# zhirui-gao/Curve-Gaussian

Hardware: AMD Instinct MI355X
Metric: Msplats rasterized/s (fwd+bwd) (higher is better)
Workload: dtype f32

## Files before the change

### curve_gaussian_amd/csrc/curve_math.h

```cpp
#pragma once
#include "kernels.h"

namespace cgs {

constexpr int NORM_SLOTS = 64;
constexpr int NQ_FWD = 3, NQ_ALL = 5;
constexpr int NORM_WORDS = NQ_ALL * NORM_SLOTS;
static_assert(NORM_WORDS <= 384, "norms buffer layout");

struct SampleCoef {
    float c[4];
    float cf[4];
    float d[3];
    float l[2];
    float lf[2];
    float pad;
};
static_assert(sizeof(SampleCoef) == 64, "SampleCoef must be 16 floats");

struct V3 { float x, y, z; };
__device__ __forceinline__ V3 operator+(V3 a, V3 b) { return {a.x + b.x, a.y + b.y, a.z + b.z}; }
__device__ __forceinline__ V3 operator-(V3 a, V3 b) { return {a.x - b.x, a.y - b.y, a.z - b.z}; }
__device__ __forceinline__ V3 operator*(float s, V3 a) { return {s * a.x, s * a.y, s * a.z}; }
__device__ __forceinline__ float dot(V3 a, V3 b) { return a.x * b.x + a.y * b.y + a.z * b.z; }
__device__ __forceinline__ V3 cross(V3 a, V3 b) { return {a.y * b.z - a.z * b.y, a.z * b.x - a.x * b.z, a.x * b.y - a.y * b.x}; }

struct CurveCP { V3 p0, p1, p2, p3; bool bez; };
__device__ __forceinline__ CurveCP load_curve(const float* __restrict__ cp, const uint8_t* __restrict__ is_bezier, int b) {
    const float4* q = reinterpret_cast<const float4*>(cp + (size_t)b * 12);
    const float4 a = q[0], c = q[1], d = q[2];
    CurveCP r;
    r.p0 = {a.x, a.y, a.z}; r.p1 = {a.w, c.x, c.y}; r.p2 = {c.z, c.w, d.x}; r.p3 = {d.y, d.z, d.w};
    r.bez = is_bezier ? (is_bezier[b] != 0) : true;
    return r;
}
__device__ __forceinline__ V3 curve_tangent(const CurveCP& c, const SampleCoef& k) {
    if (!c.bez) return c.p3 - c.p0;
    return k.d[0] * (c.p1 - c.p0) + k.d[1] * (c.p2 - c.p1) + k.d[2] * (c.p3 - c.p2);
}

struct BlockConst {
    float N1, N2, D2, D1;
};
__device__ __forceinline__ void stage_consts(const SampleCoef* __restrict__ coef, int m, const double* __restrict__ norms,
                                             SampleCoef* s_coef, BlockConst* s_bc) {
    const float* src = reinterpret_cast<const float*>(coef);
    float* dst = reinterpret_cast<float*>(s_coef);
    for (int t = threadIdx.x; t < m * 16; t += blockDim.x) dst[t] = src[t];
    __shared__ double s_q[NQ_ALL];
    for (int base = 0; base < NQ_ALL * NORM_SLOTS; base += blockDim.x) {
        const int idx = base + threadIdx.x;
        double v = idx < NQ_ALL * NORM_SLOTS ? norms[idx] : 0.0;
#pragma unroll
        for (int off = NORM_SLOTS / 2; off >= 1; off >>= 1) v += __shfl_xor(v, off, 64);
        if (idx < NQ_ALL * NORM_SLOTS && (idx % NORM_SLOTS) == 0) s_q[idx / NORM_SLOTS] = v;
    }
    __syncthreads();
    if (threadIdx.x == 0) {
        const double N1 = sqrt(s_q[0]), N2 = sqrt(s_q[1]) / N1;
        s_bc->N1 = (float)N1;
        s_bc->N2 = (float)N2;
        s_bc->D2 = (float)s_q[3];
        s_bc->D1 = (float)(s_q[4] - s_q[3] / (N2 * N2 * N2) * (s_q[2] / N1));
    }
    __syncthreads();
}
constexpr int SAMPLE_BLOCK = 256;
constexpr int MAX_M = 32;

struct CurveLaunch { int cpb; dim3 grid; };
inline CurveLaunch curve_launch(int B, int m) {
    const int cpb = SAMPLE_BLOCK / m;
    return {cpb, dim3((B + cpb - 1) / cpb)};
}
struct CurveSlot { int i, b; bool valid; };
__device__ __forceinline__ CurveSlot curve_slot(int B, int m, int curves_per_block) {
    const int lc = threadIdx.x / m;
    CurveSlot t;
    t.i = threadIdx.x - lc * m;
    t.b = blockIdx.x * curves_per_block + lc;
    t.valid = lc < curves_per_block && t.b < B;
    return t;
}

template <int N>
__device__ __forceinline__ void block_accumulate(const double (&v)[N], double* norms, int q0) {
    __shared__ double s_part[N][4];
    double w[N];
#pragma unroll
    for (int k = 0; k < N; k++) w[k] = (double)wave_sum((float)v[k]);
    const int wave = threadIdx.x >> 6;
    if ((threadIdx.x & 63) == 0) {
#pragma unroll
        for (int k = 0; k < N; k++) s_part[k][wave] = w[k];
    }
    __syncthreads();
    if (threadIdx.x < N) {
        double t = 0;
        for (int wv = 0; wv < (int)(blockDim.x >> 6); wv++) t += s_part[threadIdx.x][wv];
        atomicAdd(norms + (q0 + threadIdx.x) * NORM_SLOTS + (blockIdx.x % NORM_SLOTS), t);
    }
}

struct QuatFwd { float a[4], qa[4], N[4], D; int k; bool flip; };
__device__ __forceinline__ float sel4(const float (&arr)[4], int k) {
    return k == 0 ? arr[0] : (k == 1 ? arr[1] : (k == 2 ? arr[2] : arr[3]));
}
__device__ __forceinline__ QuatFwd quat_forward(const float M[3][3], float q[4]) {
    QuatFwd f;
    const float m00 = M[0][0], m01 = M[0][1], m02 = M[0][2], m10 = M[1][0], m11 = M[1][1], m12 = M[1][2], m20 = M[2][0],
                m21 = M[2][1], m22 = M[2][2];
    f.a[0] = 1.0f + m00 + m11 + m22; f.a[1] = 1.0f + m00 - m11 - m22;
    f.a[2] = 1.0f - m00 + m11 - m22; f.a[3] = 1.0f - m00 - m11 + m22;
    int k = 0;
#pragma unroll
    for (int j = 0; j < 4; j++) f.qa[j] = f.a[j] > 0.f ? sqrtf(f.a[j]) : 0.f;
    float qak = f.qa[0];
#pragma unroll
    for (int j = 1; j < 4; j++) {
        const bool gt = f.qa[j] > qak;
        k = gt ? j : k;
        qak = gt ? f.qa[j] : qak;
    }
    f.k = k;
    const float sq = qak * qak;
    if (k == 0) { f.N[0] = sq; f.N[1] = m21 - m12; f.N[2] = m02 - m20; f.N[3] = m10 - m01; }
    else if (k == 1) { f.N[0] = m21 - m12; f.N[1] = sq; f.N[2] = m10 + m01; f.N[3] = m02 + m20; }
    else if (k == 2) { f.N[0] = m02 - m20; f.N[1] = m10 + m01; f.N[2] = sq; f.N[3] = m12 + m21; }
    else { f.N[0] = m10 - m01; f.N[1] = m20 + m02; f.N[2] = m21 + m12; f.N[3] = sq; }
    f.D = 2.0f * fmaxf(qak, 0.1f);
#pragma unroll
    for (int j = 0; j < 4; j++) q[j] = f.N[j] / f.D;
    f.flip = q[0] < 0.f;
    if (f.flip) {
#pragma unroll
        for (int j = 0; j < 4; j++) q[j] = -q[j];
    }
    return f;
}
__device__ __forceinline__ void quat_backward(const QuatFwd& f, const float g_out[4], float gM[3][3]) {
    float gc[4], gN[4];
    float gD = 0.f;
#pragma unroll
    for (int j = 0; j < 4; j++) {
        gc[j] = f.flip ? -g_out[j] : g_out[j];
        gN[j] = gc[j] / f.D;
        gD -= gc[j] * f.N[j] / (f.D * f.D);
    }
    const int k = f.k;
    const float qak = sel4(f.qa, k);
    const float g_qa = (qak > 0.1f ? 2.f * gD : 0.f) + sel4(gN, k) * 2.f * qak;
    const float g_a = sel4(f.a, k) > 0.f ? g_qa / (2.f * qak) : 0.f;
#pragma unroll
    for (int r = 0; r < 3; r++)
#pragma unroll
        for (int c = 0; c < 3; c++) gM[r][c] = 0.f;
    const float s00 = (k == 0 || k == 1) ? 1.f : -1.f, s11 = (k == 0 || k == 2) ? 1.f : -1.f,
                s22 = (k == 0 || k == 3) ? 1.f : -1.f;
    gM[0][0] = s00 * g_a; gM[1][1] = s11 * g_a; gM[2][2] = s22 * g_a;
    if (k == 0) {
        gM[2][1] += gN[1]; gM[1][2] -= gN[1]; gM[0][2] += gN[2]; gM[2][0] -= gN[2]; gM[1][0] += gN[3]; gM[0][1] -= gN[3];
    } else if (k == 1) {
        gM[2][1] += gN[0]; gM[1][2] -= gN[0]; gM[1][0] += gN[2]; gM[0][1] += gN[2]; gM[0][2] += gN[3]; gM[2][0] += gN[3];
    } else if (k == 2) {
        gM[0][2] += gN[0]; gM[2][0] -= gN[0]; gM[1][0] += gN[1]; gM[0][1] += gN[1]; gM[1][2] += gN[3]; gM[2][1] += gN[3];
    } else {
        gM[1][0] += gN[0]; gM[0][1] -= gN[0]; gM[2][0] += gN[1]; gM[0][2] += gN[1]; gM[2][1] += gN[2]; gM[1][2] += gN[2];
    }
}

struct SampleFwd {
    V3 xyz, dvec, tan, v0, c1v, v1, c2v, v2;
    float dist, n;
};
__device__ __forceinline__ SampleFwd sample_forward(const CurveCP& c, const SampleCoef& k, float N1, float N2, float eps) {
    SampleFwd s;
    V3 front;
    if (c.bez) {
        s.xyz = k.c[0] * c.p0 + k.c[1] * c.p1 + k.c[2] * c.p2 + k.c[3] * c.p3;
        front = k.cf[0] * c.p0 + k.cf[1] * c.p1 + k.cf[2] * c.p2 + k.cf[3] * c.p3;
    } else {
        s.xyz = k.l[0] * c.p0 + k.l[1] * c.p3;
        front = k.lf[0] * c.p0 + k.lf[1] * c.p3;
    }
    s.dvec = s.xyz - front;
    s.dist = sqrtf(dot(s.dvec, s.dvec));
    s.tan = curve_tangent(c, k);
    s.n = sqrtf(dot(s.tan, s.tan));
    s.v0 = {s.tan.x / (s.n + eps), s.tan.y / (s.n + eps), s.tan.z / (s.n + eps)};
    s.c1v = {s.tan.y, -s.tan.x, 0.f};
    s.v1 = {s.c1v.x / N1, s.c1v.y / N1, 0.f};
    s.c2v = cross(s.tan, s.v1);
    s.v2 = {s.c2v.x / N2, s.c2v.y / N2, s.c2v.z / N2};
    return s;
}
__device__ __forceinline__ void rot_matrix(const SampleFwd& s, float M[3][3]) {
    M[0][0] = s.v0.x; M[0][1] = s.v1.x; M[0][2] = s.v2.x;
    M[1][0] = s.v0.y; M[1][1] = s.v1.y; M[1][2] = s.v2.y;
    M[2][0] = s.v0.z; M[2][1] = s.v1.z; M[2][2] = s.v2.z;
}

struct NormTerms { double d2, a; };
__device__ __forceinline__ NormTerms norm_sum_terms(const SampleFwd& s, float N2, V3 g_v1, V3 g_v2) {
    NormTerms t;
    t.d2 = (double)dot(g_v2, s.c2v);
    t.a = (double)dot(g_v1, s.c1v) + (double)((1.f / N2) * dot(cross(g_v2, s.tan), s.c1v));
    return t;
}

struct CurveGrad { V3 gp0, gp1, gp2, gp3; float gw; };
__device__ __forceinline__ CurveGrad sample_backward_tail(const CurveCP& c, const SampleCoef& k, const SampleFwd& s, float w, float eps,
                                                          float N1, float N2, float D2, float D1, V3 g_v0, V3 g_v1, V3 g_v2, V3 g_x,
                                                          bool has_scaling, V3 g_scl) {
    CurveGrad o;
    o.gp0 = o.gp1 = o.gp2 = o.gp3 = V3{0.f, 0.f, 0.f};
    o.gw = 0.f;
    const float iN2 = 1.f / N2;
    const V3 g_c2v = iN2 * g_v2 - (D2 * iN2 * iN2 * iN2) * s.c2v;
    V3 g_tan = cross(s.v1, g_c2v);
    const V3 g_v1t = g_v1 + cross(g_c2v, s.tan);
    const float iN1 = 1.f / N1;
    const V3 g_c1v = iN1 * g_v1t - (D1 * iN1 * iN1 * iN1) * s.c1v;
    g_tan.y += g_c1v.x;
    g_tan.x -= g_c1v.y;
    if (s.n > 0.f) {
        const float ne = s.n + eps;
        const float coefv = dot(g_v0, s.tan) / (s.n * ne * ne);
        g_tan = g_tan + (1.f / ne) * g_v0 - coefv * s.tan;
    } else {
        g_tan = g_tan + (1.f / eps) * g_v0;
    }
    V3 g_front = {0, 0, 0};
    if (has_scaling) {
        const float gd = g_scl.x;
        o.gw = (g_scl.y + g_scl.z) * w;
        if (s.dist > 0.f) {
            const V3 gdv = (gd / s.dist) * s.dvec;
            g_x = g_x + gdv;
            g_front = {-gdv.x, -gdv.y, -gdv.z};
        }
    }
    if (c.bez) {
        o.gp0 = k.c[0] * g_x + k.cf[0] * g_front - k.d[0] * g_tan;
        o.gp1 = k.c[1] * g_x + k.cf[1] * g_front + (k.d[0] - k.d[1]) * g_tan;
        o.gp2 = k.c[2] * g_x + k.cf[2] * g_front + (k.d[1] - k.d[2]) * g_tan;
        o.gp3 = k.c[3] * g_x + k.cf[3] * g_front + k.d[2] * g_tan;
    } else {
        o.gp0 = k.l[0] * g_x + k.lf[0] * g_front - g_tan;
        o.gp3 = k.l[1] * g_x + k.lf[1] * g_front + g_tan;
    }
    return o;
}
constexpr int CURVE_PART = 13;
template <typename F>
__device__ __forceinline__ void curve_reduce(const CurveGrad& g, float (*s_part)[256 + 1], int B, int m, int curves_per_block, F fn) {
    const int t = threadIdx.x;
    s_part[0][t] = g.gp0.x; s_part[1][t] = g.gp0.y; s_part[2][t] = g.gp0.z;
    s_part[3][t] = g.gp1.x; s_part[4][t] = g.gp1.y; s_part[5][t] = g.gp1.z;
    s_part[6][t] = g.gp2.x; s_part[7][t] = g.gp2.y; s_part[8][t] = g.gp2.z;
    s_part[9][t] = g.gp3.x; s_part[10][t] = g.gp3.y; s_part[11][t] = g.gp3.z;
    s_part[12][t] = g.gw;
    __syncthreads();
    for (int o = threadIdx.x; o < curves_per_block * CURVE_PART; o += blockDim.x) {
        const int c2 = o / CURVE_PART, f = o - c2 * CURVE_PART;
        float sum = 0.f;
        for (int q = 0; q < m; q++) sum += s_part[f][c2 * m + q];
        const int bb = blockIdx.x * curves_per_block + c2;
        if (bb < B) fn(bb, f, sum);
    }
}
__device__ __forceinline__ void store_curve_grad(float* __restrict__ g_cp, float* __restrict__ g_width, int bb, int f, float v,
                                                 int accumulate) {
    float* dst = f < 12 ? g_cp + (size_t)bb * 12 + f : g_width + bb;
    *dst = accumulate ? *dst + v : v;
}

__device__ __forceinline__ float sigmoidf_(float x) { return 1.f / (1.f + expf(-x)); }

struct AttrsFwd { float4 rot_n; float opac, mk; float4 all_map; float nrm; };
__device__ __forceinline__ AttrsFwd attrs_forward(const float4 q, const V3 x, float opacity_logit, bool has_mask,
                                                  float mask_logit, float mask_thr, const V3 cam,
                                                  const float* __restrict__ vm) {
    AttrsFwd o;
    const float op = sigmoidf_(opacity_logit);
    o.nrm = sqrtf(q.x * q.x + q.y * q.y + q.z * q.z + q.w * q.w);
    const float den = fmaxf(o.nrm, 1e-12f);
    const float r = q.x / den, qi = q.y / den, qj = q.z / den, qk = q.w / den;
    o.rot_n = make_float4(r, qi, qj, qk);
    o.mk = 1.f;
    if (has_mask) o.mk = sigmoidf_(mask_logit) > mask_thr ? 1.f : 0.f;
    o.opac = op * o.mk;
    const float two_s = 2.0f / (r * r + qi * qi + qj * qj + qk * qk);
    V3 d = {1.f - two_s * (qj * qj + qk * qk), two_s * (qi * qj + qk * r), two_s * (qi * qk - qj * r)};
    if (dot(d, cam - x) < 0.0f) d = {-d.x, -d.y, -d.z};
    o.all_map = make_float4(d.x * vm[0] + d.y * vm[4] + d.z * vm[8], d.x * vm[1] + d.y * vm[5] + d.z * vm[9],
                            d.x * vm[2] + d.y * vm[6] + d.z * vm[10], 1.0f);
    return o;
}

struct AttrsBwd { float4 g_rot_raw; float g_op_term, g_mask_logit, mk; };
__device__ __forceinline__ AttrsBwd attrs_backward(const float4 q, const V3 x, float opacity_logit, bool has_mask,
                                                   float mask_logit, float mask_thr, const V3 cam,
                                                   const float* __restrict__ vm, float4 gqn, bool has_ga, const float4 ga,
                                                   float go, bool has_gs, const V3 gs, const V3 scaling) {
    AttrsBwd o;
    const float op = sigmoidf_(opacity_logit);
    const float nrm = sqrtf(q.x * q.x + q.y * q.y + q.z * q.z + q.w * q.w);
    const float den = fmaxf(nrm, 1e-12f);
    const float r = q.x / den, qi = q.y / den, qj = q.z / den, qk = q.w / den;
    float gq[4] = {gqn.x, gqn.y, gqn.z, gqn.w};
    if (has_ga) {
        V3 gd = {vm[0] * ga.x + vm[1] * ga.y + vm[2] * ga.z, vm[4] * ga.x + vm[5] * ga.y + vm[6] * ga.z,
                 vm[8] * ga.x + vm[9] * ga.y + vm[10] * ga.z};
        const float s2 = r * r + qi * qi + qj * qj + qk * qk;
        const float two_s = 2.0f / s2;
        const V3 d = {1.f - two_s * (qj * qj + qk * qk), two_s * (qi * qj + qk * r), two_s * (qi * qk - qj * r)};
        if (dot(d, cam - x) < 0.0f) gd = {-gd.x, -gd.y, -gd.z};
        const float e0 = qj * qj + qk * qk, e1 = qi * qj + qk * r, e2 = qi * qk - qj * r;
        const float g_two_s = -gd.x * e0 + gd.y * e1 + gd.z * e2;
        const float g_s2 = g_two_s * (-2.0f / (s2 * s2));
        gq[0] += two_s * (gd.y * qk - gd.z * qj) + g_s2 * 2.f * r;
        gq[1] += two_s * (gd.y * qj + gd.z * qk) + g_s2 * 2.f * qi;
        gq[2] += two_s * (-2.f * gd.x * qj + gd.y * qi - gd.z * r) + g_s2 * 2.f * qj;
        gq[3] += two_s * (-2.f * gd.x * qk + gd.y * r + gd.z * qi) + g_s2 * 2.f * qk;
    }
    if (nrm > 1e-12f) {
        const float dq = gq[0] * r + gq[1] * qi + gq[2] * qj + gq[3] * qk;
        o.g_rot_raw = make_float4((gq[0] - r * dq) / nrm, (gq[1] - qi * dq) / nrm, (gq[2] - qj * dq) / nrm, (gq[3] - qk * dq) / nrm);
    } else {
        o.g_rot_raw = make_float4(gq[0] / 1e-12f, gq[1] / 1e-12f, gq[2] / 1e-12f, gq[3] / 1e-12f);
    }
    float sg = 0.f;
    o.mk = 1.f;
    if (has_mask) {
        sg = sigmoidf_(mask_logit);
        o.mk = sg > mask_thr ? 1.f : 0.f;
    }
    o.g_op_term = go * o.mk * op * (1.f - op);
    float g_mask = go * op;
    if (has_gs) g_mask += gs.x * scaling.x + gs.y * scaling.y + gs.z * scaling.z;
    o.g_mask_logit = has_mask ? g_mask * sg * (1.f - sg) : 0.f;
    return o;
}

__device__ __forceinline__ void quat_grad_to_axes(const SampleFwd& s, const float4 gq, V3& g_v0, V3& g_v1, V3& g_v2) {
    float M[3][3], q[4], gM[3][3];
    rot_matrix(s, M);
    const QuatFwd f = quat_forward(M, q);
    const float go[4] = {gq.x, gq.y, gq.z, gq.w};
    quat_backward(f, go, gM);
    g_v0 = {gM[0][0], gM[1][0], gM[2][0]};
    g_v1 = {gM[0][1], gM[1][1], gM[2][1]};
    g_v2 = {gM[0][2], gM[1][2], gM[2][2]};
}

}
```

### curve_gaussian_amd/csrc/sampling.hip

```cpp
#include <algorithm>

#include "curve_math.h"

namespace cgs {

constexpr int F12_BLOCK = 1024;
__global__ void __launch_bounds__(F12_BLOCK) k_sample_f12(int B, int m, const float* __restrict__ cp,
                                                         const uint8_t* __restrict__ is_bezier,
                                                         const SampleCoef* __restrict__ coef, double* __restrict__ norms) {
    __shared__ SampleCoef s_coef[MAX_M];
    __shared__ double s_part[3][F12_BLOCK / 64];
    const float* src = reinterpret_cast<const float*>(coef);
    float* dst = reinterpret_cast<float*>(s_coef);
    for (int t = threadIdx.x; t < m * 16; t += blockDim.x) dst[t] = src[t];
    __syncthreads();
    double a1 = 0, a2 = 0, a3 = 0;
    for (int p = blockIdx.x * blockDim.x + threadIdx.x; p < B * m; p += gridDim.x * blockDim.x) {
        const int b = p / m, i = p - b * m;
        const CurveCP c = load_curve(cp, is_bezier, b);
        const V3 t = curve_tangent(c, s_coef[i]);
        const V3 c1 = {t.y, -t.x, 0.f};
        const V3 x = cross(t, c1);
        a1 += (double)(t.y * t.y + t.x * t.x);
        a2 += (double)(x.x * x.x + x.y * x.y + x.z * x.z);
        a3 += (double)dot(cross(x, t), c1);
    }
#pragma unroll
    for (int off = 32; off >= 1; off >>= 1) {
        a1 += __shfl_xor(a1, off, 64);
        a2 += __shfl_xor(a2, off, 64);
        a3 += __shfl_xor(a3, off, 64);
    }
    if ((threadIdx.x & 63) == 0) {
        s_part[0][threadIdx.x >> 6] = a1; s_part[1][threadIdx.x >> 6] = a2; s_part[2][threadIdx.x >> 6] = a3;
    }
    __syncthreads();
    if (threadIdx.x < 3) {
        double t = 0;
        for (int wv = 0; wv < (int)(blockDim.x >> 6); wv++) t += s_part[threadIdx.x][wv];
        norms[threadIdx.x * NORM_SLOTS + blockIdx.x] = t;
    } else if (threadIdx.x < NQ_ALL) {
        norms[threadIdx.x * NORM_SLOTS + blockIdx.x] = 0.0;
    }
}

__global__ void __launch_bounds__(256) k_sample_f3(int B, int m, const float* __restrict__ cp,
                                                   const float* __restrict__ width,
                                                   const uint8_t* __restrict__ is_bezier,
                                                   const SampleCoef* __restrict__ coef, float eps,
                                                   const double* __restrict__ norms, float* __restrict__ xyz,
                                                   float* __restrict__ rot, float* __restrict__ scaling) {
    __shared__ SampleCoef s_coef[MAX_M];
    __shared__ BlockConst s_bc;
    stage_consts(coef, m, norms, s_coef, &s_bc);
    const int p = blockIdx.x * blockDim.x + threadIdx.x;
    if (p >= B * m) return;
    const int b = p / m, i = p - b * m;
    const float N1 = s_bc.N1, N2 = s_bc.N2;
    const CurveCP c = load_curve(cp, is_bezier, b);
    const float w = expf(width[b]);
    const SampleFwd s = sample_forward(c, s_coef[i], N1, N2, eps);
    float M[3][3], q[4];
    rot_matrix(s, M);
    quat_forward(M, q);
    xyz[3 * p] = s.xyz.x; xyz[3 * p + 1] = s.xyz.y; xyz[3 * p + 2] = s.xyz.z;
    reinterpret_cast<float4*>(rot)[p] = make_float4(q[0], q[1], q[2], q[3]);
    scaling[3 * p] = s.dist; scaling[3 * p + 1] = w; scaling[3 * p + 2] = w;
}

__global__ void __launch_bounds__(SAMPLE_BLOCK) k_sample_bwd_sums(int B, int m, const float* __restrict__ cp,
                                                                  const uint8_t* __restrict__ is_bezier,
                                                                  const SampleCoef* __restrict__ coef, float eps,
                                                                  double* __restrict__ norms, const float* __restrict__ g_rot,
                                                                  float* __restrict__ gv_cache) {
    __shared__ SampleCoef s_coef[MAX_M];
    __shared__ BlockConst s_bc;
    stage_consts(coef, m, norms, s_coef, &s_bc);
    const int p = blockIdx.x * blockDim.x + threadIdx.x;
    NormTerms t = {0, 0};
    if (g_rot && p < B * m) {
        const int b = p / m, i = p - b * m;
        const SampleFwd s = sample_forward(load_curve(cp, is_bezier, b), s_coef[i], s_bc.N1, s_bc.N2, eps);
        V3 g_v0, g_v1, g_v2;
        quat_grad_to_axes(s, reinterpret_cast<const float4*>(g_rot)[p], g_v0, g_v1, g_v2);
        float* gv = gv_cache + p;
        const size_t PS = (size_t)B * m;
        gv[0] = g_v0.x; gv[PS] = g_v0.y; gv[2 * PS] = g_v0.z; gv[3 * PS] = g_v1.x; gv[4 * PS] = g_v1.y; gv[5 * PS] = g_v1.z;
        gv[6 * PS] = g_v2.x; gv[7 * PS] = g_v2.y; gv[8 * PS] = g_v2.z;
        t = norm_sum_terms(s, s_bc.N2, g_v1, g_v2);
    }
    const double acc[2] = {t.d2, t.a};
    block_accumulate<2>(acc, norms, 3);
}

__global__ void __launch_bounds__(SAMPLE_BLOCK) k_sample_bwd_curves(int B, int m, int curves_per_block,
                                                                    const float* __restrict__ cp,
                                                                    const float* __restrict__ width,
                                                                    const uint8_t* __restrict__ is_bezier,
                                                                    const SampleCoef* __restrict__ coef, float eps,
                                                                    const double* __restrict__ norms,
                                                                    const float* __restrict__ g_xyz, bool has_rot,
                                                                    const float* __restrict__ g_scaling,
                                                                    float* __restrict__ g_cp, float* __restrict__ g_width,
                                                                    const float* __restrict__ gv_cache) {
    __shared__ float s_part[CURVE_PART][SAMPLE_BLOCK + 1];
    __shared__ SampleCoef s_coef[MAX_M];
    __shared__ BlockConst s_bc;
    stage_consts(coef, m, norms, s_coef, &s_bc);
    const CurveSlot t = curve_slot(B, m, curves_per_block);
    CurveGrad cg = {};
    if (t.valid) {
        const CurveCP c = load_curve(cp, is_bezier, t.b);
        const SampleCoef k = s_coef[t.i];
        const size_t p = (size_t)t.b * m + t.i;
        const SampleFwd s = sample_forward(c, k, s_bc.N1, s_bc.N2, eps);
        V3 g_v0 = {0, 0, 0}, g_v1 = {0, 0, 0}, g_v2 = {0, 0, 0}, g_x = {0, 0, 0}, g_s = {0, 0, 0};
        if (has_rot) {
            const float* gv = gv_cache + p;
            const size_t PS = (size_t)B * m;
            g_v0 = {gv[0], gv[PS], gv[2 * PS]}; g_v1 = {gv[3 * PS], gv[4 * PS], gv[5 * PS]}; g_v2 = {gv[6 * PS], gv[7 * PS], gv[8 * PS]};
        }
        if (g_xyz) g_x = {g_xyz[3 * p], g_xyz[3 * p + 1], g_xyz[3 * p + 2]};
        if (g_scaling) g_s = {g_scaling[3 * p], g_scaling[3 * p + 1], g_scaling[3 * p + 2]};
        cg = sample_backward_tail(c, k, s, expf(width[t.b]), eps, s_bc.N1, s_bc.N2, s_bc.D2, s_bc.D1, g_v0, g_v1, g_v2, g_x,
                                  g_scaling != nullptr, g_s);
    }
    curve_reduce(cg, s_part, B, m, curves_per_block, [&](int bb, int f, float sum) { store_curve_grad(g_cp, g_width, bb, f, sum, 0); });
}

__global__ void __launch_bounds__(SAMPLE_BLOCK) k_sample_bwd_close(int B, int m, int curves_per_block, const float* __restrict__ cp,
                                                                   const float* __restrict__ width,
                                                                   const uint8_t* __restrict__ is_bezier,
                                                                   const SampleCoef* __restrict__ coef, float eps,
                                                                   const double* __restrict__ norms, const float* __restrict__ part,
                                                                   float* __restrict__ g_cp, float* __restrict__ g_width,
                                                                   int accumulate) {
    __shared__ float s_part[CURVE_PART][SAMPLE_BLOCK + 1];
    __shared__ SampleCoef s_coef[MAX_M];
    __shared__ BlockConst s_bc;
    stage_consts(coef, m, norms, s_coef, &s_bc);
    const CurveSlot t = curve_slot(B, m, curves_per_block);
    CurveGrad cg = {};
    if (t.valid) {
        const CurveCP c = load_curve(cp, is_bezier, t.b);
        const SampleCoef k = s_coef[t.i];
        const SampleFwd s = sample_forward(c, k, s_bc.N1, s_bc.N2, eps);
        const V3 z = {0.f, 0.f, 0.f};
        cg = sample_backward_tail(c, k, s, expf(width[t.b]), eps, s_bc.N1, s_bc.N2, s_bc.D2, s_bc.D1, z, z, z, z, false, z);
    }
    curve_reduce(cg, s_part, B, m, curves_per_block, [&](int bb, int f, float sum) {
        store_curve_grad(g_cp, g_width, bb, f, part[(size_t)bb * CURVE_PART + f] + sum, accumulate);
    });
}


__global__ void __launch_bounds__(256) k_attrs_fwd(int B, int m, const float* __restrict__ rot_raw,
                                                   const float* __restrict__ xyz,
                                                   const float* __restrict__ opacity_logit,
                                                   const float* __restrict__ mask_logit, float mask_thr,
                                                   const float* __restrict__ scaling,
                                                   const float* __restrict__ campos, const float* __restrict__ vm,
                                                   float* __restrict__ rot_n, float* __restrict__ opac,
                                                   float* __restrict__ scl_out, float* __restrict__ all_map) {
    const int p = blockIdx.x * blockDim.x + threadIdx.x;
    if (p >= B * m) return;
    const int b = p / m;
    const V3 cam = {campos[0], campos[1], campos[2]};
    const float4 q = reinterpret_cast<const float4*>(rot_raw)[p];
    const V3 x = {xyz[3 * p], xyz[3 * p + 1], xyz[3 * p + 2]};
    const AttrsFwd a = attrs_forward(q, x, opacity_logit[b], mask_logit != nullptr, mask_logit ? mask_logit[p] : 0.f, mask_thr,
                                     cam, vm);
    reinterpret_cast<float4*>(rot_n)[p] = a.rot_n;
    opac[p] = a.opac;
    if (scl_out) {
        scl_out[3 * p] = scaling[3 * p] * a.mk; scl_out[3 * p + 1] = scaling[3 * p + 1] * a.mk;
        scl_out[3 * p + 2] = scaling[3 * p + 2] * a.mk;
    }
    reinterpret_cast<float4*>(all_map)[p] = a.all_map;
}

__global__ void __launch_bounds__(SAMPLE_BLOCK) k_attrs_bwd(
    int B, int m, int curves_per_block, const float* __restrict__ rot_raw, const float* __restrict__ xyz,
    const float* __restrict__ opacity_logit, const float* __restrict__ mask_logit, float mask_thr,
    const float* __restrict__ scaling, const float* __restrict__ campos, const float* __restrict__ vm,
    const float* __restrict__ g_rot_n, const float* __restrict__ g_opac, const float* __restrict__ g_scl_out,
    const float* __restrict__ g_all_map, float* __restrict__ g_rot_raw, float* __restrict__ g_opacity_logit,
    float* __restrict__ g_mask_logit, float* __restrict__ g_scaling) {
    __shared__ float s_go[SAMPLE_BLOCK];
    const CurveSlot t = curve_slot(B, m, curves_per_block);
    const int b = t.b;
    float g_op_term = 0.f;
    if (t.valid) {
        const size_t p = (size_t)b * m + t.i;
        const V3 cam = {campos[0], campos[1], campos[2]};
        const float4 q = reinterpret_cast<const float4*>(rot_raw)[p];
        const V3 x = {xyz[3 * p], xyz[3 * p + 1], xyz[3 * p + 2]};
        const float4 gqn = g_rot_n ? reinterpret_cast<const float4*>(g_rot_n)[p] : make_float4(0.f, 0.f, 0.f, 0.f);
        const float4 ga = g_all_map ? reinterpret_cast<const float4*>(g_all_map)[p] : make_float4(0.f, 0.f, 0.f, 0.f);
        V3 gs = {0.f, 0.f, 0.f}, sc = {0.f, 0.f, 0.f};
        if (g_scl_out) {
            gs = {g_scl_out[3 * p], g_scl_out[3 * p + 1], g_scl_out[3 * p + 2]};
            sc = {scaling[3 * p], scaling[3 * p + 1], scaling[3 * p + 2]};
        }
        const AttrsBwd o = attrs_backward(q, x, opacity_logit[b], mask_logit != nullptr, mask_logit ? mask_logit[p] : 0.f,
                                          mask_thr, cam, vm, gqn, g_all_map != nullptr, ga, g_opac ? g_opac[p] : 0.f,
                                          g_scl_out != nullptr, gs, sc);
        reinterpret_cast<float4*>(g_rot_raw)[p] = o.g_rot_raw;
        g_op_term = o.g_op_term;
        if (g_scl_out && g_scaling) { g_scaling[3 * p] = gs.x * o.mk; g_scaling[3 * p + 1] = gs.y * o.mk; g_scaling[3 * p + 2] = gs.z * o.mk; }
        if (g_mask_logit) g_mask_logit[p] = o.g_mask_logit;
    }
    s_go[threadIdx.x] = g_op_term;
    __syncthreads();
    if (t.valid && t.i == 0) {
        float sum = 0.f;
        for (int q = 0; q < m; q++) sum += s_go[threadIdx.x + q];
        g_opacity_logit[b] = sum;
    }
}

static int f12_threads(long long P) { return P <= 128 * 1024 ? 256 : (P <= 600 * 1024 ? 512 : 1024); }

void launch_sample_norms(hipStream_t s, int B, int m, const float* cp, const uint8_t* is_bezier, const void* coef, double* norms) {
    ProfScope p("sample_f12", s);
    hipLaunchKernelGGL(k_sample_f12, dim3(NORM_SLOTS), dim3(f12_threads((long long)B * m)), 0, s, B, m, cp, is_bezier,
                       reinterpret_cast<const SampleCoef*>(coef), norms);
}
void launch_sample_forward(hipStream_t s, int B, int m, const float* cp, const float* width, const uint8_t* is_bezier,
                           const void* coef, float eps, double* norms, float* xyz, float* rot, float* scaling) {
    launch_sample_norms(s, B, m, cp, is_bezier, coef, norms);
    ProfScope p("sample_f3", s);
    hipLaunchKernelGGL(k_sample_f3, dim3((B * m + 255) / 256), dim3(256), 0, s, B, m, cp, width, is_bezier,
                       reinterpret_cast<const SampleCoef*>(coef), eps, norms, xyz, rot, scaling);
}
void launch_sample_backward(hipStream_t s, int B, int m, const float* cp, const float* width, const uint8_t* is_bezier,
                            const void* coef, float eps, double* norms, const float* g_xyz, const float* g_rot,
                            const float* g_scaling, float* g_cp, float* g_width, float* gv_cache) {
    const CurveLaunch cl = curve_launch(B, m);
    const dim3 block(SAMPLE_BLOCK), sgrid(std::max((B * m + SAMPLE_BLOCK - 1) / SAMPLE_BLOCK, 1));
    const SampleCoef* k = reinterpret_cast<const SampleCoef*>(coef);
    { ProfScope p("sample_b1", s); hipLaunchKernelGGL(k_sample_bwd_sums, sgrid, block, 0, s, B, m, cp, is_bezier, k, eps, norms, g_rot, gv_cache); }
    { ProfScope p("sample_b3", s); hipLaunchKernelGGL(k_sample_bwd_curves, cl.grid, block, 0, s, B, m, cl.cpb, cp, width, is_bezier, k, eps, norms, g_xyz, g_rot != nullptr, g_scaling, g_cp, g_width, gv_cache); }
}
void launch_attrs_forward(hipStream_t s, int B, int m, const float* rot_raw, const float* xyz, const float* opacity_logit,
                          const float* mask_logit, float mask_thr, const float* scaling, const float* campos,
                          const float* vm, float* rot_n, float* opac, float* scl_out, float* all_map) {
    ProfScope p("attrs_fwd", s);
    hipLaunchKernelGGL(k_attrs_fwd, dim3((B * m + 255) / 256), dim3(256), 0, s, B, m, rot_raw, xyz, opacity_logit, mask_logit,
                       mask_thr, scaling, campos, vm, rot_n, opac, scl_out, all_map);
}
void launch_attrs_backward(hipStream_t s, int B, int m, const float* rot_raw, const float* xyz,
                           const float* opacity_logit, const float* mask_logit, float mask_thr, const float* scaling,
                           const float* campos, const float* vm, const float* g_rot_n, const float* g_opac,
                           const float* g_scl_out, const float* g_all_map, float* g_rot_raw, float* g_opacity_logit,
                           float* g_mask_logit, float* g_scaling) {
    ProfScope p("attrs_bwd", s);
    const CurveLaunch cl = curve_launch(B, m);
    hipLaunchKernelGGL(k_attrs_bwd, cl.grid, dim3(SAMPLE_BLOCK), 0, s, B, m, cl.cpb, rot_raw, xyz, opacity_logit, mask_logit,
                       mask_thr, scaling, campos, vm, g_rot_n, g_opac, g_scl_out, g_all_map, g_rot_raw, g_opacity_logit,
                       g_mask_logit, g_scaling);
}

void launch_sample_backward_close(hipStream_t s, int B, int m, const float* cp, const float* width, const uint8_t* is_bezier,
                                  const void* coef, float eps, const double* norms, const float* part, float* g_cp, float* g_width,
                                  int accumulate) {
    const CurveLaunch cl = curve_launch(B, m);
    ProfScope p("sample_b3", s);
    hipLaunchKernelGGL(k_sample_bwd_close, cl.grid, dim3(SAMPLE_BLOCK), 0, s, B, m, cl.cpb, cp, width, is_bezier,
                       reinterpret_cast<const SampleCoef*>(coef), eps, norms, part, g_cp, g_width, accumulate);
}

int sample_norm_words() { return NORM_WORDS; }
int sample_norm_fwd_words() { return NQ_FWD * NORM_SLOTS; }

}
```

### curve_gaussian_amd/csrc/view.hip

```cpp
#include "curve_math.h"
#include "splat_math.h"

namespace cgs {

__global__ void __launch_bounds__(256) k_view_fwd(
    int B, int m, const float* __restrict__ cp, const float* __restrict__ width, const uint8_t* __restrict__ is_bezier,
    const SampleCoef* __restrict__ coef, float eps, const double* __restrict__ norms,
    const float* __restrict__ opacity_logit, const float* __restrict__ mask_logit, float mask_thr,
    const float* __restrict__ colors_precomp, const float* __restrict__ campos, ViewParams vp,
    float* __restrict__ xyz_out, float* __restrict__ rot_out, float* __restrict__ scl_out, int* __restrict__ radii,
    SplatRec* __restrict__ rec, float* __restrict__ grad_acc, uint32_t* __restrict__ clear_words, uint32_t n_clear) {
    __shared__ SampleCoef s_coef[MAX_M];
    __shared__ BlockConst s_bc;
    stage_consts(coef, m, norms, s_coef, &s_bc);
    const int p = blockIdx.x * blockDim.x + threadIdx.x;
    for (uint32_t i = (uint32_t)p; i < n_clear; i += gridDim.x * blockDim.x) clear_words[i] = 0u;
    if (p >= B * m) return;
    {
        float4* accp = reinterpret_cast<float4*>(grad_acc + (size_t)p * ACC_STRIDE_VIEW);
        const float4 z = make_float4(0.f, 0.f, 0.f, 0.f);
#pragma unroll
        for (int k = 0; k < ACC_STRIDE_VIEW / 4; k++) accp[k] = z;
    }
    const int b = p / m, i = p - b * m;
    const CurveCP c = load_curve(cp, is_bezier, b);
    const float w = expf(width[b]);
    const SampleFwd s = sample_forward(c, s_coef[i], s_bc.N1, s_bc.N2, eps);
    float M[3][3], q[4];
    rot_matrix(s, M);
    quat_forward(M, q);
    if (xyz_out) {
        xyz_out[3 * p] = s.xyz.x; xyz_out[3 * p + 1] = s.xyz.y; xyz_out[3 * p + 2] = s.xyz.z;
        reinterpret_cast<float4*>(rot_out)[p] = make_float4(q[0], q[1], q[2], q[3]);
        scl_out[3 * p] = s.dist; scl_out[3 * p + 1] = w; scl_out[3 * p + 2] = w;
    }
    const V3 cam = {campos[0], campos[1], campos[2]};
    const AttrsFwd a = attrs_forward(make_float4(q[0], q[1], q[2], q[3]), s.xyz, opacity_logit[b], mask_logit != nullptr,
                                     mask_logit ? mask_logit[p] : 0.f, mask_thr, cam, vp.vm);
    const float3 sc = make_float3(s.dist * a.mk, w * a.mk, w * a.mk);
    float cov3D[6];
    cov3d_from_scale_rot(sc, 1.0f, a.rot_n, cov3D);
    SplatGeom g;
    int out_radius = 0;
    if (splat_geometry(make_float3(s.xyz.x, s.xyz.y, s.xyz.z), cov3D, vp, 0, g)) {
        rec[p] = splat_record(g, a.opac, colors_precomp ? colors_precomp[p] : 1.0f, a.all_map);
        out_radius = (int)g.radius;
    }
    radii[p] = out_radius;
}

#ifndef CGS_VIEW_BWD_WAVES
#define CGS_VIEW_BWD_WAVES 6
#endif
#ifndef CGS_VIEW_BWD_WAVES_LARGE
#define CGS_VIEW_BWD_WAVES_LARGE 4
#endif
constexpr int VIEW_BWD_LARGE_P = 512 * 1024;
template <int WAVES>
__global__ void __launch_bounds__(SAMPLE_BLOCK, WAVES) k_view_bwd(
    int B, int m, int curves_per_block, const float* __restrict__ cp, const float* __restrict__ width,
    const uint8_t* __restrict__ is_bezier, const SampleCoef* __restrict__ coef, float eps, double* __restrict__ norms,
    const float* __restrict__ opacity_logit, const float* __restrict__ mask_logit, float mask_thr,
    const float* __restrict__ campos, ViewParams vp, const int* __restrict__ radii, const SplatRec* __restrict__ rec,
    float* __restrict__ grad_acc, const float* __restrict__ g_rot_raw_extra, float* __restrict__ dL_dmean2D,
    float* __restrict__ g_opacity_logit, float* __restrict__ g_mask_logit, float* __restrict__ curve_part,
    int accumulate_flags) {
    const int accumulate = accumulate_flags & 1;
    const bool acc_scr = (accumulate_flags & 2) != 0;
    __shared__ float s_part[CURVE_PART][SAMPLE_BLOCK + 1];
    __shared__ SampleCoef s_coef[MAX_M];
    __shared__ BlockConst s_bc;
    __shared__ float s_go[SAMPLE_BLOCK];
    stage_consts(coef, m, norms, s_coef, &s_bc);
    const CurveSlot t = curve_slot(B, m, curves_per_block);
    const int i = t.i, b = t.b;
    const bool valid = t.valid;
    float g_op_term = 0.f;
    NormTerms nt = {0, 0};
    CurveGrad cg;
    cg.gp0 = cg.gp1 = cg.gp2 = cg.gp3 = V3{0.f, 0.f, 0.f};
    cg.gw = 0.f;
    if (valid) {
        const size_t p = (size_t)b * m + i;
        const float N1 = s_bc.N1, N2 = s_bc.N2;
        const CurveCP c = load_curve(cp, is_bezier, b);
        const float w = expf(width[b]);
        const SampleFwd s = sample_forward(c, s_coef[i], N1, N2, eps);
        float M[3][3], qv[4];
        rot_matrix(s, M);
        const QuatFwd f = quat_forward(M, qv);
        const float4 q = make_float4(qv[0], qv[1], qv[2], qv[3]);
        const V3 cam = {campos[0], campos[1], campos[2]};
        const bool has_mask = mask_logit != nullptr;
        const float ml = has_mask ? mask_logit[p] : 0.f;
        const AttrsFwd a = attrs_forward(q, s.xyz, opacity_logit[b], has_mask, ml, mask_thr, cam, vp.vm);
        const float3 sc = make_float3(s.dist * a.mk, w * a.mk, w * a.mk);
        float4* accp = reinterpret_cast<float4*>(grad_acc + (size_t)p * ACC_STRIDE_VIEW);
        const float4 acc0 = accp[0], acc1 = accp[1];
        {
            const float4 z = make_float4(0.f, 0.f, 0.f, 0.f);
            accp[0] = z; accp[1] = z;
        }
        const bool vis = radii[p] > 0;
        float4 ra = make_float4(0.f, 0.f, 0.f, 0.f), rb = ra;
        float cov3D[6] = {0.f, 0.f, 0.f, 0.f, 0.f, 0.f};
        if (vis) {
            ra = rec[p].a;
            rb = rec[p].b;
            cov3d_from_scale_rot(sc, 1.0f, a.rot_n, cov3D);
        }
        SplatGrads o;
        splat_backward(acc0, acc1, vis, ra, rb, make_float3(s.xyz.x, s.xyz.y, s.xyz.z), cov3D, sc, a.rot_n, true, 1.0f, 0.f,
                       vp, 0, false, o);
        dL_dmean2D[3 * p] = o.g2x; dL_dmean2D[3 * p + 1] = o.g2y; dL_dmean2D[3 * p + 2] = 0.f;
        const V3 gs = {o.dscale.x, o.dscale.y, o.dscale.z};
        const V3 scl = {s.dist, w, w};
        const AttrsBwd ab = attrs_backward(q, s.xyz, opacity_logit[b], has_mask, ml, mask_thr, cam, vp.vm, o.drot, false , make_float4(0.f, 0.f, 0.f, 0.f),
                                           o.dopac, has_mask, gs, scl);
        g_op_term = ab.g_op_term;
        if (g_mask_logit) g_mask_logit[p] = accumulate ? g_mask_logit[p] + ab.g_mask_logit : ab.g_mask_logit;
        float4 grr = ab.g_rot_raw;
        if (g_rot_raw_extra) {
            const float4 e = reinterpret_cast<const float4*>(g_rot_raw_extra)[p];
            grr = make_float4(grr.x + e.x, grr.y + e.y, grr.z + e.z, grr.w + e.w);
        }
        float gM[3][3];
        const float go[4] = {grr.x, grr.y, grr.z, grr.w};
        quat_backward(f, go, gM);
        const V3 g_v0 = {gM[0][0], gM[1][0], gM[2][0]};
        const V3 g_v1 = {gM[0][1], gM[1][1], gM[2][1]};
        const V3 g_v2 = {gM[0][2], gM[1][2], gM[2][2]};
        nt = norm_sum_terms(s, N2, g_v1, g_v2);
        const V3 g_x = {o.dmean.x, o.dmean.y, o.dmean.z}, g_s = {gs.x * ab.mk, gs.y * ab.mk, gs.z * ab.mk};
        cg = sample_backward_tail(c, s_coef[i], s, w, eps, N1, N2, 0.f, 0.f, g_v0, g_v1, g_v2, g_x, true, g_s);
    }
    s_go[threadIdx.x] = g_op_term;
    const double acc2v[2] = {nt.d2, nt.a};
    block_accumulate<2>(acc2v, norms, 3);
    curve_reduce(cg, s_part, B, m, curves_per_block, [&](int bb, int f, float sum) {
        float* dst = curve_part + (size_t)bb * CURVE_PART + f;
        *dst = acc_scr ? *dst + sum : sum;
    });
    if (valid && i == 0) {
        float sum = 0.f;
        for (int k = 0; k < m; k++) sum += s_go[threadIdx.x + k];
        g_opacity_logit[b] = accumulate ? g_opacity_logit[b] + sum : sum;
    }
}

void launch_view_forward(hipStream_t s, int B, int m, const float* cp, const float* width, const uint8_t* is_bezier,
                         const void* coef, float eps, const double* norms, const float* opacity_logit,
                         const float* mask_logit, float mask_thr, const float* colors_precomp, const float* campos,
                         const float* viewmatrix, const float* projmatrix, float tan_fovx, float tan_fovy, float focal_x,
                         float focal_y, int W, int H, int grid_x, int grid_y, float* xyz, float* rot, float* scl, int* radii,
                         SplatRec* rec, float* grad_acc, uint32_t* clear_words, size_t n_clear) {
    ProfScope p("view_fwd", s);
    const ViewParams vp{viewmatrix, projmatrix, tan_fovx, tan_fovy, focal_x, focal_y, W, H, grid_x, grid_y};
    hipLaunchKernelGGL(k_view_fwd, dim3((B * m + 255) / 256), dim3(256), 0, s, B, m, cp, width, is_bezier,
                       reinterpret_cast<const SampleCoef*>(coef), eps, norms, opacity_logit, mask_logit, mask_thr,
                       colors_precomp, campos, vp, xyz, rot, scl, radii, rec, grad_acc, clear_words, (uint32_t)n_clear);
}
void launch_view_backward(hipStream_t s, int B, int m, const float* cp, const float* width, const uint8_t* is_bezier,
                          const void* coef, float eps, double* norms, const float* opacity_logit, const float* mask_logit,
                          float mask_thr, const float* campos, const float* viewmatrix, const float* projmatrix,
                          float tan_fovx, float tan_fovy, float focal_x, float focal_y, int W, int H, const int* radii,
                          const SplatRec* rec, float* grad_acc, const float* g_rot_raw_extra, float* dL_dmean2D,
                          float* g_opacity_logit, float* g_mask_logit, float* curve_part, int accumulate) {
    ProfScope p("view_bwd", s);
    const CurveLaunch cl = curve_launch(B, m);
    const ViewParams vp{viewmatrix, projmatrix, tan_fovx, tan_fovy, focal_x, focal_y, W, H, 0, 0};
    const auto launch = [&](auto kernel) {
        hipLaunchKernelGGL(kernel, cl.grid, dim3(SAMPLE_BLOCK), 0, s, B, m, cl.cpb, cp, width, is_bezier,
                           reinterpret_cast<const SampleCoef*>(coef), eps, norms, opacity_logit, mask_logit, mask_thr, campos, vp,
                           radii, rec, grad_acc, g_rot_raw_extra, dL_dmean2D, g_opacity_logit, g_mask_logit, curve_part, accumulate);
    };
    if ((long long)B * m >= VIEW_BWD_LARGE_P) launch(k_view_bwd<CGS_VIEW_BWD_WAVES_LARGE>);
    else launch(k_view_bwd<CGS_VIEW_BWD_WAVES>);
}

}
```

Measured before the change: 812.2.

## Overlap norm-reduction staging with curve loads and restructure norm sampling loop

```diff
diff --git a/curve_gaussian_amd/csrc/curve_math.h b/curve_gaussian_amd/csrc/curve_math.h
--- a/curve_gaussian_amd/csrc/curve_math.h
+++ b/curve_gaussian_amd/csrc/curve_math.h
@@ -42,28 +42,40 @@
 struct BlockConst {
     float N1, N2, D2, D1;
 };
-__device__ __forceinline__ void stage_consts(const SampleCoef* __restrict__ coef, int m, const double* __restrict__ norms,
-                                             SampleCoef* s_coef, BlockConst* s_bc) {
+template <bool WITH_D>
+__device__ __forceinline__ const double* stage_consts_begin(const SampleCoef* __restrict__ coef, int m,
+                                                            const double* __restrict__ norms, SampleCoef* s_coef) {
     const float* src = reinterpret_cast<const float*>(coef);
     float* dst = reinterpret_cast<float*>(s_coef);
     for (int t = threadIdx.x; t < m * 16; t += blockDim.x) dst[t] = src[t];
     __shared__ double s_q[NQ_ALL];
-    for (int base = 0; base < NQ_ALL * NORM_SLOTS; base += blockDim.x) {
+    constexpr int NQ = WITH_D ? NQ_ALL : 2;
+    for (int base = 0; base < NQ * NORM_SLOTS; base += blockDim.x) {
         const int idx = base + threadIdx.x;
-        double v = idx < NQ_ALL * NORM_SLOTS ? norms[idx] : 0.0;
+        double v = idx < NQ * NORM_SLOTS ? norms[idx] : 0.0;
 #pragma unroll
         for (int off = NORM_SLOTS / 2; off >= 1; off >>= 1) v += __shfl_xor(v, off, 64);
-        if (idx < NQ_ALL * NORM_SLOTS && (idx % NORM_SLOTS) == 0) s_q[idx / NORM_SLOTS] = v;
+        if (idx < NQ * NORM_SLOTS && (idx % NORM_SLOTS) == 0) s_q[idx / NORM_SLOTS] = v;
     }
     __syncthreads();
+    return s_q;
+}
+template <bool WITH_D>
+__device__ __forceinline__ void stage_consts_finish(const double* s_q, BlockConst* s_bc) {
     if (threadIdx.x == 0) {
         const double N1 = sqrt(s_q[0]), N2 = sqrt(s_q[1]) / N1;
         s_bc->N1 = (float)N1;
         s_bc->N2 = (float)N2;
-        s_bc->D2 = (float)s_q[3];
-        s_bc->D1 = (float)(s_q[4] - s_q[3] / (N2 * N2 * N2) * (s_q[2] / N1));
+        if (WITH_D) {
+            s_bc->D2 = (float)s_q[3];
+            s_bc->D1 = (float)(s_q[4] - s_q[3] / (N2 * N2 * N2) * (s_q[2] / N1));
+        }
     }
     __syncthreads();
+}
+__device__ __forceinline__ void stage_consts(const SampleCoef* __restrict__ coef, int m, const double* __restrict__ norms,
+                                             SampleCoef* s_coef, BlockConst* s_bc) {
+    stage_consts_finish<true>(stage_consts_begin<true>(coef, m, norms, s_coef), s_bc);
 }
 constexpr int SAMPLE_BLOCK = 256;
 constexpr int MAX_M = 32;
@@ -173,7 +185,7 @@
     V3 xyz, dvec, tan, v0, c1v, v1, c2v, v2;
     float dist, n;
 };
-__device__ __forceinline__ SampleFwd sample_forward(const CurveCP& c, const SampleCoef& k, float N1, float N2, float eps) {
+__device__ __forceinline__ SampleFwd sample_forward_local(const CurveCP& c, const SampleCoef& k, float eps) {
     SampleFwd s;
     V3 front;
     if (c.bez) {
@@ -189,9 +201,16 @@
     s.n = sqrtf(dot(s.tan, s.tan));
     s.v0 = {s.tan.x / (s.n + eps), s.tan.y / (s.n + eps), s.tan.z / (s.n + eps)};
     s.c1v = {s.tan.y, -s.tan.x, 0.f};
+    return s;
+}
+__device__ __forceinline__ void sample_forward_norms(SampleFwd& s, float N1, float N2) {
     s.v1 = {s.c1v.x / N1, s.c1v.y / N1, 0.f};
     s.c2v = cross(s.tan, s.v1);
     s.v2 = {s.c2v.x / N2, s.c2v.y / N2, s.c2v.z / N2};
+}
+__device__ __forceinline__ SampleFwd sample_forward(const CurveCP& c, const SampleCoef& k, float N1, float N2, float eps) {
+    SampleFwd s = sample_forward_local(c, k, eps);
+    sample_forward_norms(s, N1, N2);
     return s;
 }
 __device__ __forceinline__ void rot_matrix(const SampleFwd& s, float M[3][3]) {
diff --git a/curve_gaussian_amd/csrc/sampling.hip b/curve_gaussian_amd/csrc/sampling.hip
--- a/curve_gaussian_amd/csrc/sampling.hip
+++ b/curve_gaussian_amd/csrc/sampling.hip
@@ -15,15 +15,18 @@
     for (int t = threadIdx.x; t < m * 16; t += blockDim.x) dst[t] = src[t];
     __syncthreads();
     double a1 = 0, a2 = 0, a3 = 0;
-    for (int p = blockIdx.x * blockDim.x + threadIdx.x; p < B * m; p += gridDim.x * blockDim.x) {
-        const int b = p / m, i = p - b * m;
+    const int per = (B + (int)gridDim.x - 1) / (int)gridDim.x;
+    const int b_end = min(B, ((int)blockIdx.x + 1) * per);
+    for (int b = blockIdx.x * per + threadIdx.x; b < b_end; b += blockDim.x) {
         const CurveCP c = load_curve(cp, is_bezier, b);
-        const V3 t = curve_tangent(c, s_coef[i]);
-        const V3 c1 = {t.y, -t.x, 0.f};
-        const V3 x = cross(t, c1);
-        a1 += (double)(t.y * t.y + t.x * t.x);
-        a2 += (double)(x.x * x.x + x.y * x.y + x.z * x.z);
-        a3 += (double)dot(cross(x, t), c1);
+        for (int i = 0; i < m; i++) {
+            const V3 t = curve_tangent(c, s_coef[i]);
+            const V3 c1 = {t.y, -t.x, 0.f};
+            const V3 x = cross(t, c1);
+            a1 += (double)(t.y * t.y + t.x * t.x);
+            a2 += (double)(x.x * x.x + x.y * x.y + x.z * x.z);
+            a3 += (double)dot(cross(x, t), c1);
+        }
     }
 #pragma unroll
     for (int off = 32; off >= 1; off >>= 1) {
@@ -138,15 +141,19 @@
     __shared__ float s_part[CURVE_PART][SAMPLE_BLOCK + 1];
     __shared__ SampleCoef s_coef[MAX_M];
     __shared__ BlockConst s_bc;
-    stage_consts(coef, m, norms, s_coef, &s_bc);
     const CurveSlot t = curve_slot(B, m, curves_per_block);
+    const int b = t.valid ? t.b : 0;
+    const CurveCP c = load_curve(cp, is_bezier, b);
+    const float wl = width[b];
+    const double* s_q = stage_consts_begin<true>(coef, m, norms, s_coef);
+    const SampleCoef k = s_coef[t.i];
+    SampleFwd s = sample_forward_local(c, k, eps);
+    stage_consts_finish<true>(s_q, &s_bc);
     CurveGrad cg = {};
     if (t.valid) {
-        const CurveCP c = load_curve(cp, is_bezier, t.b);
-        const SampleCoef k = s_coef[t.i];
-        const SampleFwd s = sample_forward(c, k, s_bc.N1, s_bc.N2, eps);
+        sample_forward_norms(s, s_bc.N1, s_bc.N2);
         const V3 z = {0.f, 0.f, 0.f};
-        cg = sample_backward_tail(c, k, s, expf(width[t.b]), eps, s_bc.N1, s_bc.N2, s_bc.D2, s_bc.D1, z, z, z, z, false, z);
+        cg = sample_backward_tail(c, k, s, expf(wl), eps, s_bc.N1, s_bc.N2, s_bc.D2, s_bc.D1, z, z, z, z, false, z);
     }
     curve_reduce(cg, s_part, B, m, curves_per_block, [&](int bb, int f, float sum) {
         store_curve_grad(g_cp, g_width, bb, f, part[(size_t)bb * CURVE_PART + f] + sum, accumulate);
diff --git a/curve_gaussian_amd/csrc/view.hip b/curve_gaussian_amd/csrc/view.hip
--- a/curve_gaussian_amd/csrc/view.hip
+++ b/curve_gaussian_amd/csrc/view.hip
@@ -12,20 +12,26 @@
     SplatRec* __restrict__ rec, float* __restrict__ grad_acc, uint32_t* __restrict__ clear_words, uint32_t n_clear) {
     __shared__ SampleCoef s_coef[MAX_M];
     __shared__ BlockConst s_bc;
-    stage_consts(coef, m, norms, s_coef, &s_bc);
     const int p = blockIdx.x * blockDim.x + threadIdx.x;
-    for (uint32_t i = (uint32_t)p; i < n_clear; i += gridDim.x * blockDim.x) clear_words[i] = 0u;
-    if (p >= B * m) return;
-    {
+    const bool valid = p < B * m;
+    const int b = valid ? p / m : 0, i = p - (p / m) * m;
+    const CurveCP c = load_curve(cp, is_bezier, b);
+    const float wl = width[b], ol = opacity_logit[b];
+    const float ml = mask_logit && valid ? mask_logit[p] : 0.f;
+    const float col = colors_precomp && valid ? colors_precomp[p] : 1.0f;
+    const double* s_q = stage_consts_begin<false>(coef, m, norms, s_coef);
+    for (uint32_t j = (uint32_t)p; j < n_clear; j += gridDim.x * blockDim.x) clear_words[j] = 0u;
+    if (valid) {
         float4* accp = reinterpret_cast<float4*>(grad_acc + (size_t)p * ACC_STRIDE_VIEW);
         const float4 z = make_float4(0.f, 0.f, 0.f, 0.f);
 #pragma unroll
         for (int k = 0; k < ACC_STRIDE_VIEW / 4; k++) accp[k] = z;
     }
-    const int b = p / m, i = p - b * m;
-    const CurveCP c = load_curve(cp, is_bezier, b);
-    const float w = expf(width[b]);
-    const SampleFwd s = sample_forward(c, s_coef[i], s_bc.N1, s_bc.N2, eps);
+    const float w = expf(wl);
+    SampleFwd s = sample_forward_local(c, s_coef[i], eps);
+    stage_consts_finish<false>(s_q, &s_bc);
+    if (!valid) return;
+    sample_forward_norms(s, s_bc.N1, s_bc.N2);
     float M[3][3], q[4];
     rot_matrix(s, M);
     quat_forward(M, q);
@@ -35,15 +41,14 @@
         scl_out[3 * p] = s.dist; scl_out[3 * p + 1] = w; scl_out[3 * p + 2] = w;
     }
     const V3 cam = {campos[0], campos[1], campos[2]};
-    const AttrsFwd a = attrs_forward(make_float4(q[0], q[1], q[2], q[3]), s.xyz, opacity_logit[b], mask_logit != nullptr,
-                                     mask_logit ? mask_logit[p] : 0.f, mask_thr, cam, vp.vm);
+    const AttrsFwd a = attrs_forward(make_float4(q[0], q[1], q[2], q[3]), s.xyz, ol, mask_logit != nullptr, ml, mask_thr, cam, vp.vm);
     const float3 sc = make_float3(s.dist * a.mk, w * a.mk, w * a.mk);
     float cov3D[6];
     cov3d_from_scale_rot(sc, 1.0f, a.rot_n, cov3D);
     SplatGeom g;
     int out_radius = 0;
     if (splat_geometry(make_float3(s.xyz.x, s.xyz.y, s.xyz.z), cov3D, vp, 0, g)) {
-        rec[p] = splat_record(g, a.opac, colors_precomp ? colors_precomp[p] : 1.0f, a.all_map);
+        rec[p] = splat_record(g, a.opac, col, a.all_map);
         out_radius = (int)g.radius;
     }
     radii[p] = out_radius;
@@ -71,10 +76,14 @@
     __shared__ SampleCoef s_coef[MAX_M];
     __shared__ BlockConst s_bc;
     __shared__ float s_go[SAMPLE_BLOCK];
-    stage_consts(coef, m, norms, s_coef, &s_bc);
     const CurveSlot t = curve_slot(B, m, curves_per_block);
-    const int i = t.i, b = t.b;
+    const int i = t.i, b = t.valid ? t.b : 0;
     const bool valid = t.valid;
+    const CurveCP c = load_curve(cp, is_bezier, b);
+    const float wl = width[b], ol = opacity_logit[b];
+    const double* s_q = stage_consts_begin<false>(coef, m, norms, s_coef);
+    SampleFwd s = sample_forward_local(c, s_coef[i], eps);
+    stage_consts_finish<false>(s_q, &s_bc);
     float g_op_term = 0.f;
     NormTerms nt = {0, 0};
     CurveGrad cg;
@@ -83,9 +92,8 @@
     if (valid) {
         const size_t p = (size_t)b * m + i;
         const float N1 = s_bc.N1, N2 = s_bc.N2;
-        const CurveCP c = load_curve(cp, is_bezier, b);
-        const float w = expf(width[b]);
-        const SampleFwd s = sample_forward(c, s_coef[i], N1, N2, eps);
+        const float w = expf(wl);
+        sample_forward_norms(s, N1, N2);
         float M[3][3], qv[4];
         rot_matrix(s, M);
         const QuatFwd f = quat_forward(M, qv);
@@ -93,7 +101,7 @@
         const V3 cam = {campos[0], campos[1], campos[2]};
         const bool has_mask = mask_logit != nullptr;
         const float ml = has_mask ? mask_logit[p] : 0.f;
-        const AttrsFwd a = attrs_forward(q, s.xyz, opacity_logit[b], has_mask, ml, mask_thr, cam, vp.vm);
+        const AttrsFwd a = attrs_forward(q, s.xyz, ol, has_mask, ml, mask_thr, cam, vp.vm);
         const float3 sc = make_float3(s.dist * a.mk, w * a.mk, w * a.mk);
         float4* accp = reinterpret_cast<float4*>(grad_acc + (size_t)p * ACC_STRIDE_VIEW);
         const float4 acc0 = accp[0], acc1 = accp[1];
@@ -115,7 +123,7 @@
         dL_dmean2D[3 * p] = o.g2x; dL_dmean2D[3 * p + 1] = o.g2y; dL_dmean2D[3 * p + 2] = 0.f;
         const V3 gs = {o.dscale.x, o.dscale.y, o.dscale.z};
         const V3 scl = {s.dist, w, w};
-        const AttrsBwd ab = attrs_backward(q, s.xyz, opacity_logit[b], has_mask, ml, mask_thr, cam, vp.vm, o.drot, false , make_float4(0.f, 0.f, 0.f, 0.f),
+        const AttrsBwd ab = attrs_backward(q, s.xyz, ol, has_mask, ml, mask_thr, cam, vp.vm, o.drot, false , make_float4(0.f, 0.f, 0.f, 0.f),
                                            o.dopac, has_mask, gs, scl);
         g_op_term = ab.g_op_term;
         if (g_mask_logit) g_mask_logit[p] = accumulate ? g_mask_logit[p] + ab.g_mask_logit : ab.g_mask_logit;
```

Result: no change. 813.0, median of 3 (+0.1%).
